# dotchen/LAV

Measured on AMD Instinct MI355X. Metric: frames/s full agent fwd (32k-pt LiDAR + 3 cams), higher is better.
Workload: dtype f32 (convolution contractions on the matrix cores with f32 accumulate at the error of an fp32 dot product, DESIGN 4.3: the layers on the split-operand kernel - BEV backbone, heads, crop stems, the brake net's mid-size layers - and ERFNet's persistent runs of pairs as two power-of-two-scaled fp16 pie

## Files before the change

### include/lav_amd.h

```cpp
#ifndef LAV_AMD_H
#define LAV_AMD_H

#include <stddef.h>
#include <stdint.h>

#ifdef __cplusplus
extern "C" {
#endif

#define LAV_ABI_VERSION 39

#define LAV_OK 0
#define LAV_EINVAL (-1)
#define LAV_EHIP (-2)
#define LAV_EWORKSPACE (-3)

int lav_abi_version(void);
const char *lav_last_error(void);
int lav_device_count(void);

int lav_profile_enable(int slots);
int lav_profile_reset(void);
int lav_profile_read(const char *kernel, double *total_ms, int *launches);

typedef struct lav_grid {
    float min_x, max_x, min_y, max_y;
    float ppm;
    int nx, ny;
} lav_grid;

typedef struct lav_pointnet {
    const float *w1, *b1, *w2, *b2;
    int num_input;
    int channels;
} lav_pointnet;

size_t lav_pillar_workspace_bytes(int batch, int max_points, const lav_grid *grid);
int lav_pillar_workspace_init(void *workspace, size_t workspace_bytes, void *stream);

int lav_pillar_scatter(const float *points, const int *h_num_points, int batch, int max_points, int D,
                       const lav_grid *grid, const lav_pointnet *net, float *canvas,
                       int *unique_coords, int *inverse, int *counts,
                       void *workspace, size_t workspace_bytes, void *stream);
int lav_pillar_amax_count(int batch, const lav_grid *grid);
int lav_pillar_scatter_amax(const float *points, const int *h_num_points, int batch, int max_points, int D,
                            const lav_grid *grid, const lav_pointnet *net, float *canvas,
                            int *unique_coords, int *inverse, int *counts, float *amax_parts,
                            void *workspace, size_t workspace_bytes, void *stream);

typedef struct lav_camera {
    float K[9];
    float l2w[16];
    float w2c[16];
} lav_camera;

int lav_paint(const float *lidar, int n, int lidar_dim, const float *sem, int ncam, int sem_c, int h, int w,
              const lav_camera *h_cams, float *fused, int *uvz, void *stream);

int lav_gru_cast(const float *embd, int B, int embd_dim, int H, int num_cmds, int T,
                 const float *w_ih, const float *w_hh, const float *b_ih, const float *b_hh,
                 const float *mlp_w, const float *mlp_b, float *out,
                 void *workspace, size_t workspace_bytes, void *stream);
size_t lav_gru_cast_workspace_bytes(int B, int embd_dim, int H, int num_cmds, int T);
// ... 136 lines not shown
int lav_bn_train_amax_count(int batch, int channels, long plane);
int lav_bn_train_forward_amax(const float *x, const float *residual, float *y, int batch, int channels, long plane, const float *gamma,
                              const float *beta, double eps, int relu_pre, int relu_post, float *save_mean, float *save_var,
                              float *save_rstd, float *amax_y, void *workspace, size_t workspace_bytes, void *stream);
int lav_bn_train_backward_amax(const float *x, const float *y, const float *dy, int batch, int channels, long plane, const float *gamma,
                               const float *save_mean, const float *save_rstd, int relu_pre, int relu_post, float *dx, float *dres,
                               float *dgamma, float *dbeta, float *amax_dx, void *workspace, size_t workspace_bytes, void *stream);

int lav_bn_train_forward_mask(const float *x, const float *residual, const float *chmask, float *y, int batch, int channels, long plane,
                              const float *gamma, const float *beta, double eps, int relu_post, float *save_mean, float *save_var,
                              float *save_rstd, float *amax_y, void *workspace, size_t workspace_bytes, void *stream);
int lav_bn_train_backward_mask(const float *x, const float *y, const float *dy, const float *chmask, int batch, int channels, long plane,
                               const float *gamma, const float *save_mean, const float *save_rstd, int relu_post, float *dx, float *dres,
                               float *dgamma, float *dbeta, float *amax_dx, void *workspace, size_t workspace_bytes, void *stream);

size_t lav_conv_wgrad_workspace_bytes(int batch, int cin, int cout, int h, int w, int ksize, int stride);
int lav_conv_wgrad(const float *x, const float *dy, int batch, int cin, int cout, int h, int w, int ksize, int stride, float *dw,
                   void *workspace, size_t workspace_bytes, void *stream);
int lav_conv_wgrad_amax(const float *x, const float *dy, int batch, int cin, int cout, int h, int w, int ksize, int stride, float *dw,
                        void *workspace, size_t workspace_bytes, const float *amax_x, int n_amax_x, const float *amax_dy, int n_amax_dy,
                        void *stream);

size_t lav_upconv_pointwise_packed_floats(int cin, int cout, int k);
int lav_upconv_pointwise_pack(int cin, int cout, int k, const float *h_weight, float *h_packed);
int lav_upconv_pointwise_parts(int batch, int cin, int cout, int ih, int iw, int k, int pad, int out_pad);
int lav_upconv_pointwise(int batch, int cin, int cout, int ih, int iw, int k, int pad, int out_pad, const float *x, const float *w_packed,
                         const float *scale, const float *shift, int relu_pre, int out_c_total, int out_c_offset, float *y,
                         float *amax_out, void *stream);

size_t lav_conv1d_pair_packed_weight_floats(int channels);
int lav_conv1d_pair_pack_weights(int channels, const float *h_weight, float *h_packed);
size_t lav_conv1d_pair_chain_workspace_bytes(int batch, int h);
size_t lav_conv1d_pair_chain_lds_bytes(int channels, int w, int d_b_max);
int lav_conv1d_pair_chain(int batch, int channels, int h, int w, int npairs, const int *d_a, const int *d_b, const int *residual,
                          const int *relu_post, const float *x, const float *const *wa_packed, const float *const *bias_a,
                          const float *const *wb_packed, const float *const *bias_b, const float *const *scale,
                          const float *const *shift, float *const *out, void *workspace, size_t workspace_bytes, void *stream);
int lav_conv1d_pair_chain_f16(int batch, int channels, int h, int w, int npairs, const int *d_a, const int *d_b, const int *residual,
                              const int *relu_post, const float *x, const float *const *wa_packed, const float *const *bias_a,
                              const float *const *wb_packed, const float *const *bias_b, const float *const *scale,
                              const float *const *shift, float *const *out, void *workspace, size_t workspace_bytes, void *stream);
int lav_conv1d_pair_chain_region(int row_offset, int clean_rows);
int lav_conv1d_pair_chain_status(const void *workspace, int *h_timeouts_launches2, void *stream);
size_t lav_conv1d_pair_lds_bytes(int channels, int w, int d_b);
size_t lav_conv3x3_run_f16_workspace_bytes(int channels, int h, int w, int nlayers);
size_t lav_conv3x3_run_f16_lds_bytes(int channels, int h, int w);
size_t lav_conv3x3_run_f16_weight_bytes(int channels);
int lav_conv3x3_run_f16_amax_count(int channels, int h, int w);
long lav_conv_f16_weights_offset(const lav_conv *c);
int lav_conv3x3_run_f16(int channels, int h, int w, int nlayers, const float *x, const void *const *w_f16, const float *const *scale,
                        const float *const *shift, float *out, const float *amax_in, int amax_in_count, float *amax_out, void *workspace,
                        size_t workspace_bytes, void *stream);
int lav_conv3x3_run_f16_status(const void *workspace, int *h_timeouts_launches2, void *stream);
int lav_conv1d_pair(int batch, int channels, int h, int w, int d_a, int d_b, const float *x, const float *wa_packed,
                    const float *bias_a, const float *wb_packed, const float *bias_b, const float *scale, const float *shift,
                    const float *residual, int relu_post, float *y, void *stream);

int lav_pool_affine(const float *x, int batch, int channels, int h, int w, const float *scale, const float *shift, int relu,
                    float *y, int out_c_total, int out_c_offset, void *stream);

int lav_pair_train_supported(int channels, int width);
size_t lav_pair_train_workspace_bytes(int batch, int channels, int h);
int lav_pair_train_forward(const float *x, const float *wa, const float *ba, const float *wb, const float *bb, int batch, int channels,
                           int h, int w, int dil, float *t, float *z, void *stream);
int lav_pair_train_backward(const float *x, const float *t, const float *dz, const float *wa, const float *wb, int batch, int channels,
                            int h, int w, int dil, float *dt, float *dx, float *dwa, float *dba, float *dwb, float *dbb, void *workspace,
                            size_t workspace_bytes, void *stream);

size_t lav_seg_xent_workspace_bytes(void);
int lav_seg_xent_forward(const float *logits, const long long *labels, int batch, int classes, long plane, float *loss, float *dlogits,
                         void *workspace, size_t workspace_bytes, void *stream);

int lav_seg_xent_up_forward(const float *logits, const void *labels, int label_bytes, int batch, int classes, int h, int w, int scale,
                            float *loss, float *dlogits, void *workspace, size_t workspace_bytes, void *stream);

typedef struct lav_camera_f64 {
    double l2w[16];
    double w2c[16];
    double K[9];
} lav_camera_f64;

int lav_paint_frames(const float *lidar, const int *offsets, int frames, int total, int lidar_dim, const float *sem, int ncam,
                     int sem_c, int h, int w, const lav_camera_f64 *h_cams, float *painted, int *uvz, void *stream);

int lav_image_u8_to_f32(const unsigned char *img, int n, int h, int w, int c_src, int reverse, float *out, void *stream);

enum { LAV_AUG_BLUR = 0, LAV_AUG_NOISE = 1, LAV_AUG_DROPOUT = 2, LAV_AUG_MULTIPLY = 3, LAV_AUG_CONTRAST = 4, LAV_AUG_GRAYSCALE = 5,
       LAV_AUG_ELASTIC = 6, LAV_AUG_OPS = 7 };

typedef struct lav_augment_params {
    int order[7];
    int active;
    int per_channel;
    unsigned sample;
    unsigned tag;
    float blur_sigma;
    float blur_w[5];
    float noise_scale;
    float dropout_p;
    float multiply[3];
    float contrast[3];
    float gray_alpha;
    float elastic_alpha;
    float field_w[5];
} lav_augment_params;

// ... 39 lines not shown
```

### lav_amd/_lib.py

```python
from __future__ import annotations

import ctypes as C
import os

HERE = os.path.dirname(os.path.abspath(__file__))
LIB_PATH = os.environ.get("LAV_AMD_LIB") or os.path.join(HERE, "liblav_amd.so")

ABI_VERSION = 39
MAX_CAM = 4
MAX_CAM_F64 = 8


class Grid(C.Structure):
    _fields_ = [("min_x", C.c_float), ("max_x", C.c_float), ("min_y", C.c_float), ("max_y", C.c_float),
                ("ppm", C.c_float), ("nx", C.c_int), ("ny", C.c_int)]


class PointNet(C.Structure):
    _fields_ = [("w1", C.c_void_p), ("b1", C.c_void_p), ("w2", C.c_void_p), ("b2", C.c_void_p),
                ("num_input", C.c_int), ("channels", C.c_int)]


class Camera(C.Structure):
    _fields_ = [("K", C.c_float * 9), ("l2w", C.c_float * 16), ("w2c", C.c_float * 16)]


class CameraF64(C.Structure):
    _fields_ = [("l2w", C.c_double * 16), ("w2c", C.c_double * 16), ("K", C.c_double * 9)]


class Conv(C.Structure):
    _fields_ = [(n, C.c_int) for n in (
        "batch", "in_c_total", "in_c_offset", "cin", "h", "w", "cout", "kh", "kw", "stride", "pad_h", "pad_w",
        "dil_h", "dil_w", "transposed", "out_pad", "out_c_total", "out_c_offset", "relu_pre", "relu_post", "sigmoid", "target_cus")] + [("pad_value", C.c_float), ("precision", C.c_int)]


CONV_F32, CONV_BF16X6, CONV_F16X3 = 1, 2, 3


_P, _I, _Z, _F = C.c_void_p, C.c_int, C.c_size_t, C.c_float
SIGNATURES = {
    "lav_abi_version": (_I, []),
    "lav_last_error": (C.c_char_p, []),
    "lav_device_count": (_I, []),
    "lav_profile_enable": (_I, [_I]),
    "lav_profile_reset": (_I, []),
    "lav_profile_read": (_I, [C.c_char_p, C.POINTER(C.c_double), C.POINTER(_I)]),
    "lav_pillar_workspace_bytes": (_Z, [_I, _I, C.POINTER(Grid)]),
    "lav_pillar_workspace_init": (_I, [_P, _Z, _P]),
    "lav_pillar_decorate_workspace_bytes": (_Z, [_I, _I, C.POINTER(Grid)]),
    "lav_pillar_scatter": (_I, [_P, C.POINTER(_I), _I, _I, _I, C.POINTER(Grid), C.POINTER(PointNet), _P, _P, _P, _P,
                                _P, _Z, _P]),
    "lav_pillar_amax_count": (_I, [_I, C.POINTER(Grid)]),
    "lav_pillar_scatter_amax": (_I, [_P, C.POINTER(_I), _I, _I, _I, C.POINTER(Grid), C.POINTER(PointNet), _P, _P, _P, _P, _P,
                                     _P, _Z, _P]),
    "lav_paint": (_I, [_P, _I, _I, _P, _I, _I, _I, _I, C.POINTER(Camera), _P, _P, _P]),
    "lav_paint_frames": (_I, [_P, _P, _I, _I, _I, _P, _I, _I, _I, _I, C.POINTER(CameraF64), _P, _P, _P]),
    "lav_image_u8_to_f32": (_I, [_P, _I, _I, _I, _I, _I, _P, _P]),
    "lav_gru_cast": (_I, [_P, _I, _I, _I, _I, _I, _P, _P, _P, _P, _P, _P, _P, _P, _Z, _P]),
    "lav_gru_cast_workspace_bytes": (_Z, [_I, _I, _I, _I, _I]),
    "lav_embed_cast": (_I, [_P, _I, _I, _I, _P, _I, _I, _I, _P, _P, _P, _P, _P, _P, _P, _P, _P, _P, _P, _P, _P]),
    "lav_gru_plan": (_I, [_P, _P, _P, _I, _I, _I, _I, _I, _I, _F, _F, _P, _P, _P, _P, _P, _P, _P, _P, _Z, _P]),
    "lav_gru_plan_steps": (_I, [_P, _P, _P, _I, _I, _I, _I, _I, _I, _F, _F, _P, _P, _P, _P, _P, _P, _P, _P, _Z, _P]),
    "lav_gru_plan_status": (_I, [_P, _Z, _I, _I, _I, _I, C.POINTER(_I), _P]),
    "lav_gru_plan_diag": (_I, [_P, _Z, _I, _I, _I, _I, C.POINTER(_I), _P]),
    "lav_gru_plan_workspace_bytes": (_Z, [_I, _I, _I, _I]),
    "lav_conv_out_hw": (_I, [C.POINTER(Conv), C.POINTER(_I), C.POINTER(_I)]),
    "lav_conv_packed_weight_floats": (_Z, [C.POINTER(Conv)]),
    "lav_conv_pack_weights": (_I, [C.POINTER(Conv), _P, _P]),
    "lav_conv_pack_map_ints": (_Z, [C.POINTER(Conv)]),
    "lav_conv_pack_map": (_I, [C.POINTER(Conv), _P]),
    "lav_conv_repack": (_I, [C.POINTER(Conv), _P, _P, _P, _P]),
    "lav_conv_repack_scratch": (_I, [C.POINTER(Conv), _P, _P, _P, _P, _Z, _P]),
    "lav_bn_fold": (_I, [_P, _P, _P, _P, C.c_double, _I, _P, _P, _P]),
    "lav_conv_wgrad_workspace_bytes": (_Z, [_I, _I, _I, _I, _I, _I, _I]),
    "lav_conv_wgrad": (_I, [_P, _P, _I, _I, _I, _I, _I, _I, _I, _P, _P, _Z, _P]),
    "lav_conv_wgrad_amax": (_I, [_P, _P, _I, _I, _I, _I, _I, _I, _I, _P, _P, _Z, _P, _I, _P, _I, _P]),
    "lav_absmax_parts": (_I, [_P, C.c_long, _P, _P]),
    "lav_conv_tile_info": (_I, [C.POINTER(Conv), C.POINTER(_I)]),
    "lav_conv_workspace_bytes": (_Z, [C.POINTER(Conv)]),
    "lav_conv2d": (_I, [C.POINTER(Conv), _P, _P, _P, _P, _P, _P, _P, _P, _Z, _P]),
    "lav_conv_amax_count": (_I, [C.POINTER(Conv)]),
    "lav_conv2d_amax": (_I, [C.POINTER(Conv), _P, _P, _P, _P, _P, _P, _P, _P, _Z, _P, _I, _P, _P]),
    "lav_deconv_grouped": (_I, [_I, _I, _I, _I, _I, C.POINTER(_I), _I, _I, _I, _I, _P, _P, _P, _I, _P, _P]),
    "lav_crop_rotate": (_I, [_P, _I, _I, _I, _I, _P, _P, _I, _F, _I, _F, _F, _P, _P]),
    "lav_crop_rotate_indexed": (_I, [_P, _I, _P, _I, _I, _I, _P, _P, _I, _F, _I, _F, _F, _P, _P]),
    "lav_crop_rotate_backward": (_I, [_P, _I, _P, _I, _I, _I, _P, _P, _I, _F, _I, _F, _F, _P, _P]),
    "lav_pillar_decorate": (_I, [_P, C.POINTER(_I), _I, _I, _I, C.POINTER(Grid), _P, _P, _P, _P, _P, _P, _Z, _P]),
    "lav_scatter_max": (_I, [_P, _P, _I, _I, _I, _P, _P, _P]),
    "lav_scatter_max_backward": (_I, [_P, _P, _I, _I, _I, _P, _P]),
    "lav_conv1d_pair_packed_weight_floats": (_Z, [_I]),
    "lav_conv1d_pair_pack_weights": (_I, [_I, _P, _P]),
    "lav_upconv_pointwise_packed_floats": (_Z, [_I, _I, _I]),
    "lav_upconv_pointwise_pack": (_I, [_I, _I, _I, _P, _P]),
    "lav_upconv_pointwise_parts": (_I, [_I] * 8),
    "lav_upconv_pointwise": (_I, [_I] * 8 + [_P, _P, _P, _P, _I, _I, _I, _P, _P, _P]),
    "lav_conv1d_pair_chain_workspace_bytes": (_Z, [_I, _I]),
    "lav_conv1d_pair_chain_region": (_I, [_I, _I]),
    "lav_conv1d_pair_chain_lds_bytes": (_Z, [_I, _I, _I]),
    "lav_conv1d_pair_chain": (_I, [_I, _I, _I, _I, _I, C.POINTER(_I), C.POINTER(_I), C.POINTER(_I), C.POINTER(_I), _P] + [C.POINTER(_P)] * 7 + [_P, _Z, _P]),
    "lav_conv1d_pair_chain_f16": (_I, [_I, _I, _I, _I, _I, C.POINTER(_I), C.POINTER(_I), C.POINTER(_I), C.POINTER(_I), _P] + [C.POINTER(_P)] * 7 + [_P, _Z, _P]),
    "lav_conv1d_pair_chain_status": (_I, [_P, C.POINTER(_I), _P]),
    "lav_conv1d_pair_lds_bytes": (_Z, [_I, _I, _I]),
    "lav_conv3x3_run_f16_workspace_bytes": (_Z, [_I, _I, _I, _I]),
    "lav_conv3x3_run_f16_lds_bytes": (_Z, [_I, _I, _I]),
    "lav_conv3x3_run_f16_weight_bytes": (_Z, [_I]),
    "lav_conv3x3_run_f16_amax_count": (_I, [_I, _I, _I]),
    "lav_conv_f16_weights_offset": (C.c_long, [C.POINTER(Conv)]),
    "lav_conv3x3_run_f16": (_I, [_I, _I, _I, _I, _P, C.POINTER(_P), C.POINTER(_P), C.POINTER(_P), _P, _P, _I, _P, _P, _Z, _P]),
    "lav_conv3x3_run_f16_status": (_I, [_P, C.POINTER(_I), _P]),
    "lav_conv1d_pair": (_I, [_I, _I, _I, _I, _I, _I, _P, _P, _P, _P, _P, _P, _P, _P, _I, _P, _P]),
    "lav_gru_seq_forward": (_I, [_P, _I, _P, _P, _P, _I, _I, _I, _P, _P, _P]),
    "lav_gru_seq_backward_workspace_bytes": (_Z, [_I, _I]),
    "lav_gru_seq_backward": (_I, [_P, _P, _P, _P, _P, _I, _I, _I, _P, _P, _P, _P, _Z, _P]),
    "lav_bn_train_workspace_bytes": (_Z, [_I]),
    "lav_bn_train_forward_mask": (_I, [_P, _P, _P, _P, _I, _I, C.c_long, _P, _P, C.c_double, _I, _P, _P, _P, _P, _P, _Z, _P]),
    "lav_bn_train_backward_mask": (_I, [_P, _P, _P, _P, _I, _I, C.c_long, _P, _P, _P, _I, _P, _P, _P, _P, _P, _P, _Z, _P]),
    "lav_pair_train_supported": (_I, [_I, _I]),
    "lav_pair_train_workspace_bytes": (_Z, [_I, _I, _I]),
    "lav_pair_train_forward": (_I, [_P, _P, _P, _P, _P, _I, _I, _I, _I, _I, _P, _P, _P]),
    "lav_pair_train_backward": (_I, [_P, _P, _P, _P, _P, _I, _I, _I, _I, _I, _P, _P, _P, _P, _P, _P, _P, _Z, _P]),
    "lav_seg_xent_workspace_bytes": (_Z, []),
    "lav_seg_xent_forward": (_I, [_P, _P, _I, _I, C.c_long, _P, _P, _P, _Z, _P]),
    "lav_seg_xent_up_forward": (_I, [_P, _P, _I, _I, _I, _I, _I, _I, _P, _P, _P, _Z, _P]),
    "lav_attn_train_workspace_bytes": (_Z, [_I, _I, _I, _I]),
    "lav_attn_train_forward": (_I, [_P, _I, _I, _I, _I, _P, _P, _P, _P, C.c_float, _P, _P, _P, _P, _P, _P]),
    "lav_attn_train_backward": (_I, [_P, _I, _I, _I, _I, _P, _P, _P, _P, C.c_float, _P, _P, _P, _P, _P, _P, _P, _P, _P, _Z, _P]),
    "lav_bn_train_forward": (_I, [_P, _P, _P, _I, _I, C.c_long, _P, _P, C.c_double, _I, _I, _P, _P, _P, _P, _Z, _P]),
    "lav_bn_train_backward": (_I, [_P, _P, _P, _I, _I, C.c_long, _P, _P, _P, _I, _I, _P, _P, _P, _P, _P, _Z, _P]),
    "lav_bn_train_amax_count": (_I, [_I, _I, C.c_long]),
    "lav_bn_train_forward_amax": (_I, [_P, _P, _P, _I, _I, C.c_long, _P, _P, C.c_double, _I, _I, _P, _P, _P, _P, _P, _Z, _P]),
    "lav_bn_train_backward_amax": (_I, [_P, _P, _P, _I, _I, C.c_long, _P, _P, _P, _I, _I, _P, _P, _P, _P, _P, _P, _Z, _P]),
    "lav_attn_pool": (_I, [_P, _I, _I, _I, _I, _P, _P, _P, _P, _P, _P]),
    "lav_linear_act": (_I, [_P, _I, _I, _P, _P, _I, _I, _P, _P]),
    "lav_maxpool3x3s2": (_I, [_P, _I, _I, _I, _I, _P, _P]),
    "lav_channel_affine": (_I, [_P, _I, _I, C.c_long, _P, _P, _P, _P]),
    "lav_nonfinite_count": (_I, [_I, C.POINTER(_P), C.POINTER(C.c_long), _P, _P]),
    "lav_copy_many": (_I, [_I, C.POINTER(_P), C.POINTER(_P), C.POINTER(_Z), _P]),
    "lav_stage_many": (_I, [_I, C.POINTER(_P), C.POINTER(_P), C.POINTER(_I), C.POINTER(C.c_long), C.POINTER(_I), _P]),
    "lav_det_decode": (_I, [_P, _I, _I, _I] + [C.c_double] * 10 + [_P, _P, _P]),
    "lav_det_decode_report": (_I, [_P, _I, _I, _I] + [C.c_double] * 10 + [_P, _P, _P, _P, _P, _P]),
    "lav_stage_many_block": (_I, [_I, C.POINTER(_P), C.POINTER(_P), C.POINTER(_I), C.POINTER(C.c_long), C.POINTER(_I), _P, _I, _P, _P]),
    "lav_batch_limit": (_I, [_P]),
    "lav_pool_affine": (_I, [_P, _I, _I, _I, _I, _P, _P, _I, _P, _I, _I, _P]),
    "lav_merge_ticks": (_I, [_P, _P, _I, _I, _P, _P]),
    "lav_stack_sweeps": (_I, [_P, _P, _P, _P, _P, _P, _I, _I, _I, _P, _P]),
    "lav_extract_peaks_workspace_bytes": (_Z, [_I, _I, _I]),
    "lav_extract_peaks": (_I, [_P, _I, _I, _I, _I, _I, _I, _P, _I, _P, _I, _P, _P, _Z, _P]),
    "lav_augment_u8": (_I, [_P, _P, _I, _I, _I, _P, C.c_ulonglong, _P]),
    "lav_bev_stack_u8": (_I, [_P, _P, _P, _P, _I, _I, _I, _I, _P]),
    "lav_bev_stack_tile_paths": (_I, [C.POINTER(C.c_double), C.POINTER(_I), _I, _I, C.POINTER(_I)]),
    "lav_debug_view": (_I, [_P, _I, _I, _P, _I, _I, _P, _I, _I, _P, _I, _P, _I, _P, _I, _P, _P, _P, C.c_double, C.c_double, _I, C.c_double, C.c_double, _I,
                            _I, _I, _P, _P, _P]),
    "lav_log_view": (_I, [_P, _I, _P, _I, _P, _P, _I, _I, _P, _P, _I, _P, _I, _I, _P, _P]),
    "lav_eval_acc_words": (_Z, [_I]),
    "lav_eval_frame": (_I, [_P, _P, _P, _I, _I, _F, _P, _I, _P, _P, _I, _I, _I, _P, _P, _I, _P, _P, _P, _I] + [C.c_double] * 6 + [_I, _P, _P]),
    "lav_eval_seg": (_I, [_P, _P, _I, _I, _I, _I, _I, _P, _P]),
    "lav_eval_scores": (_I, [_P, _P, _I, C.c_double, _I, _P, _P]),
    "lav_eval_plans_words": (_Z, [_I]),
    "lav_eval_plans": (_I, [_P, _P, _P, _P, _P, _P, _I, _I, _I, _P, _P, _P, _I, _P, _P]),
}

_lib = None
# ... 35 lines not shown
```

### lav_amd/build.py

```python
from __future__ import annotations

import os
import subprocess
import sys
import time

HERE = os.path.dirname(os.path.abspath(__file__))
REPO = os.path.dirname(HERE)
CSRC = os.path.join(HERE, "csrc")
LIB = os.path.join(HERE, "liblav_amd.so")
SOURCES = ["misc.hip", "pillar.hip", "paint.hip", "paint_frames.hip", "gru.hip", "gru_seq.hip", "conv.hip", "conv_f16.hip", "conv_pair.hip", "conv_run.hip", "deconv.hip", "crop.hip", "frame.hip", "attn.hip", "bn_train.hip", "conv_wgrad.hip", "upconv.hip", "conv_pair_train.hip", "augment.hip", "bev_stack.hip", "debug_view.hip", "log_view.hip", "eval_metrics.hip", "eval_camera.hip", "eval_plans.hip"]
EXTRA_FLAGS = {"pillar.hip": ["-ffp-contract=off"], "paint.hip": ["-ffp-contract=off"], "paint_frames.hip": ["-ffp-contract=off"], "crop.hip": ["-ffp-contract=off"],
               "frame.hip": ["-ffp-contract=off"], "augment.hip": ["-ffp-contract=off"], "bev_stack.hip": ["-ffp-contract=off"],
               "debug_view.hip": ["-ffp-contract=off", "-fhip-fp32-correctly-rounded-divide-sqrt"],
               "log_view.hip": ["-ffp-contract=off"],
               "eval_metrics.hip": ["-ffp-contract=off"],
               "eval_plans.hip": ["-ffp-contract=off"]}
FLAGS = ["--offload-arch=gfx950", "-O3", "-std=c++17", "-fPIC", "-Wall", "-Wno-unused-function", "-fno-slp-vectorize",
         "-I", os.path.join(REPO, "include"), "-I", CSRC]


def _hipcc() -> str:
    for c in (os.environ.get("HIPCC"), "/opt/rocm/bin/hipcc", "hipcc"):
        if c and (os.path.isabs(c) and os.path.exists(c) or not os.path.isabs(c)):
            return c
    raise RuntimeError("hipcc not found")


def needs_build() -> bool:
    if not os.path.exists(LIB):
        return True
    t = os.path.getmtime(LIB)
    deps = [os.path.join(CSRC, f) for f in os.listdir(CSRC)] + [os.path.join(REPO, "include", "lav_amd.h")]
    return any(os.path.getmtime(d) > t for d in deps)


def build(force: bool = False, verbose: bool = True) -> str:
    if not force and not needs_build():
        return LIB
    objs = []
    procs = []
    os.makedirs(os.path.join(HERE, "build"), exist_ok=True)
    t0 = time.time()
    for s in SOURCES:
        o = os.path.join(HERE, "build", s.replace(".hip", ".o"))
        objs.append(o)
        cmd = [_hipcc(), *FLAGS, *EXTRA_FLAGS.get(s, []), "-c", os.path.join(CSRC, s), "-o", o]
        procs.append((s, subprocess.Popen(cmd, stdout=subprocess.PIPE, stderr=subprocess.STDOUT, text=True)))
    for s, p in procs:
        out, _ = p.communicate()
        if p.returncode != 0:
            raise RuntimeError(f"hipcc failed on {s}:\n{out}")
        if verbose and out.strip():
            print(out)
    link = [_hipcc(), "--offload-arch=gfx950", "-shared", "-fPIC", *objs, "-o", LIB]
    r = subprocess.run(link, stdout=subprocess.PIPE, stderr=subprocess.STDOUT, text=True)
    if r.returncode != 0:
        raise RuntimeError("link failed:\n" + r.stdout)
    if verbose:
        print(f"built {LIB} in {time.time() - t0:.1f}s")
    return LIB


if __name__ == "__main__":
# ... 2 lines not shown
```

### lav_amd/lidar.py

```python
from __future__ import annotations

import torch
from torch import nn
import torch.nn.functional as F

from . import _lib
from . import ops
from .ops import Amax, ConvLayer, ConvRun, GroupedDeconv, PointwiseUpconv
from .point_pillar import PointPillarNet

_NORM = dict(eps=1e-3, momentum=0.01)


def _refreshable(obj):
    if isinstance(obj, dict):
        for v in obj.values():
            yield from _refreshable(v)
    elif isinstance(obj, (list, tuple)):
        for v in obj:
            yield from _refreshable(v)
    elif hasattr(obj, "refresh"):
        yield obj


class _Engine(nn.Module):

    def _drop(self):
        object.__setattr__(self, "_eng", None)
        object.__setattr__(self, "_stale", False)

    def _mark_stale(self):
        if self.__dict__.get("_eng") is not None:
            object.__setattr__(self, "_stale", True)

    def _tensor_ids(self):
        return tuple(id(t) for t in self.parameters()) + tuple(id(t) for t in self.buffers())

    def _fresh(self, device):
        eng = self.__dict__.get("_eng")
        if eng is None or eng.get("device") != device:
            return None
        if self.__dict__.get("_stale"):
            if eng["tensor_ids"] != self._tensor_ids():
                self._drop()
                return None
            for layer in _refreshable(eng):
                layer.refresh()
            object.__setattr__(self, "_stale", False)
        return eng

    def _apply(self, fn, *a, **k):
        self._drop()
        return super()._apply(fn, *a, **k)

    def train(self, mode: bool = True):
        if mode != self.training:
            self._mark_stale()
        return super().train(mode)

    def _load_from_state_dict(self, *a, **k):
        self._mark_stale()
# ... 11 lines not shown
def _stage(cin, cout, n):
    mods = []
    for j in range(n):
        mods += [nn.Conv2d(cin if j == 0 else cout, cout, 3, 2 if j == 0 else 1, 1, bias=False),
                 nn.ReLU(inplace=True), nn.BatchNorm2d(cout, **_NORM)]
    return nn.Sequential(*mods)


def _up(cin, cout, k, s, p=0, op=0):
    return nn.Sequential(nn.ConvTranspose2d(cin, cout, k, s, p, op, bias=False), nn.ReLU(inplace=True),
                         nn.BatchNorm2d(cout, **_NORM))


class ConvBackbone(_Engine):
    def __init__(self, num_feature=64, norm_cfg=None):
        super().__init__()
        f = num_feature
        self.conv1 = _stage(f, f, 4)
        self.conv2 = _stage(f, 2 * f, 6)
        self.conv3 = _stage(2 * f, 2 * f, 6)
        self.upconv1 = _up(f, 2 * f, 1, 1)
        self.upconv2 = _up(2 * f, 2 * f, 4, 2, 1)
        self.upconv3 = _up(2 * f, 2 * f, 4, 4, 1, 2)
        self.out_channels = 6 * f
        self._drop()

    def _engine(self, device):
        prec = ops.infer_precision()
        eng = self._fresh(device) or dict(device=device)
        key = ("backbone", prec)
        if key in eng:
            return eng[key]
        def stage(seq):
            out = []
            for j in range(0, len(seq), 3):
                conv, bn = seq[j], seq[j + 2]
                out.append(ConvLayer(conv.weight, stride=conv.stride[0], padding=conv.padding, bn=_bn_tuple(bn),
                                     bn_eps=bn.eps, relu_pre=True, precision=prec, device=device))
            return out
        ups = []
        off = 0
        for seq in (self.upconv1, self.upconv2, self.upconv3):
            ct, bn = seq[0], seq[2]
            if prec == _lib.CONV_F16X3 and PointwiseUpconv.takes(ct):
                ups.append(PointwiseUpconv(ct, bn, relu_pre=True, out_c_total=self.out_channels, out_c_offset=off, device=device))
            else:
                ups.append(ConvLayer(ct.weight, stride=ct.stride[0], padding=ct.padding, transposed=True,
                                     output_padding=ct.output_padding[0], bn=_bn_tuple(bn), bn_eps=bn.eps, relu_pre=True,
                                     out_c_total=self.out_channels, out_c_offset=off, precision=prec, device=device))
            off += ct.weight.shape[1]
        eng[key] = dict(s1=stage(self.conv1), s2=stage(self.conv2), s3=stage(self.conv3), ups=ups, amax={}, f16=prec == _lib.CONV_F16X3)
        want = ops.bev_run_stages() if prec == _lib.CONV_F16X3 else ()
        eng[key]["runs"] = [ConvRun(eng[key][s][1:]) if s in want and len(eng[key][s]) > 2 else None for s in ("s1", "s2", "s3")]
        eng["tensor_ids"] = self._tensor_ids()
        object.__setattr__(self, "_eng", eng)
        return eng[key]

    def forward_train(self, x):
        from .train.hipnn import conv_relu_bn
        f1 = conv_relu_bn(self.conv1, x)
        f2 = conv_relu_bn(self.conv2, f1)
        f3 = conv_relu_bn(self.conv3, f2)
        return torch.cat([conv_relu_bn(self.upconv1, f1), conv_relu_bn(self.upconv2, f2), conv_relu_bn(self.upconv3, f3)], dim=1)

    def forward(self, x, out=None):
        if self.training:
            return self.forward_train(x)
        self._need_eval()
        e = self._engine(x.device)
        if not e["f16"]:
            feats = []
            for st in (e["s1"], e["s2"], e["s3"]):
                for layer in st:
                    x = layer(x)
                feats.append(x)
            oh, ow = e["ups"][0].out_hw(feats[0].shape[2], feats[0].shape[3])
            if out is None:
                out = torch.empty((x.shape[0], self.out_channels, oh, ow), dtype=torch.float32, device=x.device)
            for up, f in zip(e["ups"], feats):
                up(f, out=out)
            return out
        B = x.shape[0]
        key = ops.amax_key(x)
        ams = e["amax"].get(key)
        if ams is None:
            ams = e["amax"][key] = [Amax(x.device) for _ in range(len(e["s1"]) + len(e["s2"]) + len(e["s3"]) + 1)]
        stages = (e["s1"], e["s2"], e["s3"])
        feats, feat_am, am_prev, i = [], [], ops.amax_of(x), 0
        for si, st in enumerate(stages):
            run, li = e["runs"][si], 0
            while li < len(st):
                layer = st[li]
                oh, ow = layer.out_hw(x.shape[2], x.shape[3])
                runs_next = run is not None and run.takes(B, oh, ow)
                n = len(st) - 1 if runs_next and li == 1 else 1
                nxt = li + n
                readers = ([run if runs_next and nxt == 1 else st[nxt]] if nxt < len(st) else ([stages[si + 1][0]] if si + 1 < len(stages) else [])) + \
                          ([e["ups"][si]] if nxt == len(st) else [])
                am = ams[i + n - 1].reset() if any(r.uses_amax(B, oh, ow) for r in readers) else None
                x = (run if n > 1 else layer)(x, amax_in=am_prev, amax_out=am)
                am_prev, i, li = am, i + n, nxt
            feats.append(x); feat_am.append(am_prev)
        oh, ow = e["ups"][0].out_hw(feats[0].shape[2], feats[0].shape[3])
        if out is None:
            out = torch.empty((B, self.out_channels, oh, ow), dtype=torch.float32, device=x.device)
        am_out = ams[-1].reset()
# ... 111 lines not shown
```

### lav_amd/ops.py

```python
from __future__ import annotations

import ctypes as C
import os as _os
import threading as _threading
from typing import Optional, Sequence

import numpy as np
import torch

from . import _lib
from ._lib import Camera, Conv, Grid, PointNet, check

_workspaces: dict = {}


def _stream() -> int:
    return torch.cuda.current_stream().cuda_stream


def _ptr(t: Optional[torch.Tensor]) -> Optional[int]:
    return None if t is None else t.data_ptr()


def _f32c(t: torch.Tensor, name: str) -> torch.Tensor:
# ... 1118 lines not shown

class ConvRun:

    def __init__(self, layers):
        lib = _lib.load()
        layers = list(layers)
        l0 = layers[0]
        for l in layers:
            d = l.desc
            if not (d.precision == _lib.CONV_F16X3 and (d.kh, d.kw, d.stride, d.pad_h, d.pad_w, d.dil_h, d.dil_w) == (3, 3, 1, 1, 1, 1, 1)
                    and not d.transposed and l.cin == l.cout == l0.cin and l.in_c_total == l.cin and l.out_c_total == l.cout
                    and l.bias is None and l.scale is not None and d.relu_pre and not d.relu_post and not d.sigmoid and d.pad_value == 0.0):
                raise RuntimeError("ConvRun: layers must be identical conv3x3 / ReLU / BatchNorm layers packed for LAV_CONV_F16X3")
        self.layers, self.ch = layers, l0.cin
        probe = Conv.from_buffer_copy(l0.desc)
        probe.h, probe.w = 64, 64
        self._woff = int(lib.lav_conv_f16_weights_offset(C.byref(probe)))
        if self._woff < 0 or len(layers) > 8:
            raise RuntimeError("ConvRun: at most 8 layers with fp16 packed weights")
        n = len(layers)
        self._n = n

    def takes(self, B: int, h: int, w: int) -> bool:
        return B == 1 and _lib.load().lav_conv3x3_run_f16_workspace_bytes(self.ch, h, w, self._n) > 0

    def uses_amax(self, B: int, h: int, w: int) -> bool:
        return self.takes(B, h, w)

    def __call__(self, x: torch.Tensor, out: Optional[torch.Tensor] = None, amax_in: Optional["Amax"] = None,
                 amax_out: Optional["Amax"] = None) -> torch.Tensor:
        lib = _lib.load()
        x = _f32c(x, "x")
        B, ch, h, w = x.shape
        if ch != self.ch or not self.takes(B, h, w):
            raise RuntimeError(f"ConvRun: input {tuple(x.shape)} is not served (lav_conv3x3_run_f16_workspace_bytes)")
        if out is None:
            out = torch.empty_like(x)
        n = self._n
        ws = _workspace(("conv_run", id(self), ch, h, w), lib.lav_conv3x3_run_f16_workspace_bytes(ch, h, w, n), x.device)
        if amax_in is not None and amax_in.count > 0:
            a_in, n_in = amax_in.buf, amax_in.count
        else:
            a_in = _workspace(("conv_run_amax", id(self)), 512 * 4, x.device).view(torch.float32)
            n_in = 512
            check(lib.lav_absmax_parts(_ptr(x), x.numel(), _ptr(a_in), _stream()), "lav_absmax_parts")
        a_out = amax_out.take(lib.lav_conv3x3_run_f16_amax_count(ch, h, w)) if amax_out is not None else None
        pa = lambda ts: (C.c_void_p * n)(*[t if isinstance(t, int) else t.data_ptr() for t in ts])
        check(lib.lav_conv3x3_run_f16(ch, h, w, n, _ptr(x), pa([l.w.data_ptr() + 4 * self._woff for l in self.layers]),
                                      pa([l.scale for l in self.layers]), pa([l.shift for l in self.layers]), _ptr(out), _ptr(a_in), n_in,
                                      _ptr(a_out), _ptr(ws), ws.numel(), _stream()), "lav_conv3x3_run_f16")
        return out


def bev_run_status(device, stream=None):
    st = stream if stream is not None else torch.cuda.current_stream()
    device = torch.device(device)
    if device.index is None:
        device = torch.device("cuda", torch.cuda.current_device())
    tot = [0, 0]
    for (key, dev, s), ws in list(_workspaces.items()):
        if isinstance(key, tuple) and key and key[0] == "conv_run" and dev == device and s == st.cuda_stream:
            v = (C.c_int * 2)()
            check(_lib.load().lav_conv3x3_run_f16_status(_ptr(ws), v, st.cuda_stream), "lav_conv3x3_run_f16_status")
            tot[0] += int(v[0]); tot[1] += int(v[1])
    return tuple(tot)


_CU_COUNT = {}


def _cu_count(device) -> int:
    idx = torch.device(device).index
    idx = torch.cuda.current_device() if idx is None else idx
    if idx not in _CU_COUNT:
        _CU_COUNT[idx] = torch.cuda.get_device_properties(idx).multi_processor_count
    return _CU_COUNT[idx]


train_work = {"crop_rotate_backward_bytes": 0, "crop_rotate_backward_calls": 0, "gru_seq_forward_flops": 0, "gru_seq_backward_flops": 0,
              "bn_train_fwd_bytes": 0, "bn_train_bwd_bytes": 0, "conv_wgrad_flops": 0}


class _CropRotateIndexed(torch.autograd.Function):

    @staticmethod
    def forward(ctx, features, map_index, locs, oris, ppm, crop, ox, oy):
        lib = _lib.load()
        features = _f32c(features, "features")
        locs, oris = _f32c(locs.detach().reshape(-1, 2), "locs"), _f32c(oris.detach().reshape(-1), "oris")
        if map_index.dtype != torch.int32 or not map_index.is_cuda:
            raise RuntimeError("crop_rotate_indexed: map_index must be an int32 tensor in HBM")
        M, Cc, H, W = features.shape
        n = locs.shape[0]
        out = torch.empty((n, Cc, crop, crop), dtype=torch.float32, device=features.device)
        check(lib.lav_crop_rotate_indexed(_ptr(features), M, _ptr(map_index), Cc, H, W, _ptr(locs), _ptr(oris), n, float(ppm), int(crop),
                                          float(ox), float(oy), _ptr(out), _stream()), "lav_crop_rotate_indexed")
        ctx.save_for_backward(map_index, locs, oris)
        ctx.geom = (M, Cc, H, W, float(ppm), int(crop), float(ox), float(oy))
        return out

    @staticmethod
    def backward(ctx, grad_out):
        map_index, locs, oris = ctx.saved_tensors
        M, Cc, H, W, ppm, crop, ox, oy = ctx.geom
        grad_out = _f32c(grad_out, "grad_out")
        grad_feat = torch.empty((M, Cc, H, W), dtype=torch.float32, device=grad_out.device)
# ... 202 lines not shown
```

Measured before the change: 524.3.

## Fuse BEV backbone 3x3 conv stages into halo-tiled single-kernel f16 MFMA runs

Adds a new kernel that runs up to three consecutive 64-channel 3x3 conv+ReLU+BN layers on one spatial tile per workgroup. Each layer's intermediate activations stay in LDS as split fp16 pieces, and the kernel recomputes halo regions instead of writing them to global memory. The BEV backbone stages that have no persistent run assigned now use this path by default for batch 1. The aim is to cut the global-memory round trips and launches between layers. In exchange it spends extra compute on overlapping halos, uses heavy LDS and registers, and derives a per-tile amax for rescaling between layers.

```diff
diff --git a/include/lav_amd.h b/include/lav_amd.h
--- a/include/lav_amd.h
+++ b/include/lav_amd.h
@@ -8,7 +8,7 @@
 extern "C" {
 #endif
 
-#define LAV_ABI_VERSION 39
+#define LAV_ABI_VERSION 40
 
 #define LAV_OK 0
 #define LAV_EINVAL (-1)
@@ -251,6 +251,10 @@
                         const float *const *shift, float *out, const float *amax_in, int amax_in_count, float *amax_out, void *workspace,
                         size_t workspace_bytes, void *stream);
 int lav_conv3x3_run_f16_status(const void *workspace, int *h_timeouts_launches2, void *stream);
+size_t lav_conv3x3_tile_f16_lds_bytes(int channels, int h, int w, int nlayers);
+int lav_conv3x3_tile_f16_amax_count(int channels, int h, int w, int nlayers);
+int lav_conv3x3_tile_f16(int channels, int h, int w, int nlayers, const float *x, const void *const *w_f16, const float *const *scale,
+                         const float *const *shift, float *out, const float *amax_in, int amax_in_count, float *amax_out, void *stream);
 int lav_conv1d_pair(int batch, int channels, int h, int w, int d_a, int d_b, const float *x, const float *wa_packed,
                     const float *bias_a, const float *wb_packed, const float *bias_b, const float *scale, const float *shift,
                     const float *residual, int relu_post, float *y, void *stream);
diff --git a/lav_amd/_lib.py b/lav_amd/_lib.py
--- a/lav_amd/_lib.py
+++ b/lav_amd/_lib.py
@@ -6,7 +6,7 @@
 HERE = os.path.dirname(os.path.abspath(__file__))
 LIB_PATH = os.environ.get("LAV_AMD_LIB") or os.path.join(HERE, "liblav_amd.so")
 
-ABI_VERSION = 39
+ABI_VERSION = 40
 MAX_CAM = 4
 MAX_CAM_F64 = 8
 
@@ -109,6 +109,9 @@
     "lav_conv_f16_weights_offset": (C.c_long, [C.POINTER(Conv)]),
     "lav_conv3x3_run_f16": (_I, [_I, _I, _I, _I, _P, C.POINTER(_P), C.POINTER(_P), C.POINTER(_P), _P, _P, _I, _P, _P, _Z, _P]),
     "lav_conv3x3_run_f16_status": (_I, [_P, C.POINTER(_I), _P]),
+    "lav_conv3x3_tile_f16_lds_bytes": (_Z, [_I, _I, _I, _I]),
+    "lav_conv3x3_tile_f16_amax_count": (_I, [_I, _I, _I, _I]),
+    "lav_conv3x3_tile_f16": (_I, [_I, _I, _I, _I, _P, C.POINTER(_P), C.POINTER(_P), C.POINTER(_P), _P, _P, _I, _P, _P]),
     "lav_conv1d_pair": (_I, [_I, _I, _I, _I, _I, _I, _P, _P, _P, _P, _P, _P, _P, _P, _I, _P, _P]),
     "lav_gru_seq_forward": (_I, [_P, _I, _P, _P, _P, _I, _I, _I, _P, _P, _P]),
     "lav_gru_seq_backward_workspace_bytes": (_Z, [_I, _I]),
diff --git a/lav_amd/build.py b/lav_amd/build.py
--- a/lav_amd/build.py
+++ b/lav_amd/build.py
@@ -9,7 +9,7 @@
 REPO = os.path.dirname(HERE)
 CSRC = os.path.join(HERE, "csrc")
 LIB = os.path.join(HERE, "liblav_amd.so")
-SOURCES = ["misc.hip", "pillar.hip", "paint.hip", "paint_frames.hip", "gru.hip", "gru_seq.hip", "conv.hip", "conv_f16.hip", "conv_pair.hip", "conv_run.hip", "deconv.hip", "crop.hip", "frame.hip", "attn.hip", "bn_train.hip", "conv_wgrad.hip", "upconv.hip", "conv_pair_train.hip", "augment.hip", "bev_stack.hip", "debug_view.hip", "log_view.hip", "eval_metrics.hip", "eval_camera.hip", "eval_plans.hip"]
+SOURCES = ["misc.hip", "pillar.hip", "paint.hip", "paint_frames.hip", "gru.hip", "gru_seq.hip", "conv.hip", "conv_f16.hip", "conv_pair.hip", "conv_run.hip", "conv_tile.hip", "deconv.hip", "crop.hip", "frame.hip", "attn.hip", "bn_train.hip", "conv_wgrad.hip", "upconv.hip", "conv_pair_train.hip", "augment.hip", "bev_stack.hip", "debug_view.hip", "log_view.hip", "eval_metrics.hip", "eval_camera.hip", "eval_plans.hip"]
 EXTRA_FLAGS = {"pillar.hip": ["-ffp-contract=off"], "paint.hip": ["-ffp-contract=off"], "paint_frames.hip": ["-ffp-contract=off"], "crop.hip": ["-ffp-contract=off"],
                "frame.hip": ["-ffp-contract=off"], "augment.hip": ["-ffp-contract=off"], "bev_stack.hip": ["-ffp-contract=off"],
                "debug_view.hip": ["-ffp-contract=off", "-fhip-fp32-correctly-rounded-divide-sqrt"],
diff --git a/lav_amd/csrc/conv_tile.hip b/lav_amd/csrc/conv_tile.hip
--- /dev/null
+++ b/lav_amd/csrc/conv_tile.hip
@@ -0,0 +1,286 @@
+#include <cstdlib>
+#include <cstring>
+
+#include "common.hpp"
+#include "split_arith.hpp"
+
+namespace {
+using namespace lav;
+
+constexpr int TILE_C = 64, TILE_MAX_L = 3, TILE_MAX_WG = 16384;
+constexpr size_t TILE_W_BYTES = (size_t)9 * (TILE_C / 32) * (TILE_C / 16) * 2 * 1024;
+
+struct TileArgs {
+    const float *x;
+    float *out;
+    const unsigned char *w[TILE_MAX_L];
+    const float *wscale[TILE_MAX_L], *scale[TILE_MAX_L], *shift[TILE_MAX_L];
+    const float *amax_in;
+    float *amax_out;
+    int amax_in_count, H, W, tiles_x;
+};
+
+__device__ __forceinline__ void tile_load_w(const unsigned char *p, int t, u32x4 (&dst)[2]) {
+    dst[0] = *reinterpret_cast<const u32x4 *>(p + t * (TILE_C / 16) * 2048);
+    dst[1] = *reinterpret_cast<const u32x4 *>(p + t * (TILE_C / 16) * 2048 + 1024);
+}
+
+template <int NA, int RWI, int NPI>
+__device__ __forceinline__ void tile_mma(const unsigned char *in, const int (&base)[2], int half, u32x4 (&wr)[9][2], const unsigned char *w_this,
+                                         const unsigned char *w_next, f32x16 (&tot)[2]) {
+    constexpr int PIECE = 8 * NPI * 16;
+#pragma nounroll
+    for (int ch = 0; ch < TILE_C / 16; ++ch) {
+        f32x16 acc[NA];
+#pragma unroll
+        for (int j = 0; j < NA; ++j)
+#pragma unroll
+            for (int r = 0; r < 16; ++r) acc[j][r] = 0.f;
+        const unsigned char *w_refill = ch + 1 < TILE_C / 16 ? w_this + (ch + 1) * 2048 : w_next;
+        const unsigned char *bin = in + (ch * 2 + half) * NPI * 16;
+#pragma unroll
+        for (int t = 0; t < 9; ++t) {
+            const int toff = ((t / 3) * RWI + (t % 3)) * 16;
+            u32x4 b[NA][2];
+#pragma unroll
+            for (int j = 0; j < NA; ++j) {
+                b[j][0] = *reinterpret_cast<const u32x4 *>(bin + toff + base[j]);
+                b[j][1] = *reinterpret_cast<const u32x4 *>(bin + PIECE + toff + base[j]);
+            }
+#pragma unroll
+            for (int j = 0; j < NA; ++j)
+                acc[j] = __builtin_amdgcn_mfma_f32_32x32x16_f16(__builtin_bit_cast(f16x8, wr[t][1]), __builtin_bit_cast(f16x8, b[j][0]), acc[j], 0, 0, 0);
+#pragma unroll
+            for (int j = 0; j < NA; ++j)
+                acc[j] = __builtin_amdgcn_mfma_f32_32x32x16_f16(__builtin_bit_cast(f16x8, wr[t][0]), __builtin_bit_cast(f16x8, b[j][1]), acc[j], 0, 0, 0);
+#pragma unroll
+            for (int j = 0; j < NA; ++j)
+                acc[j] = __builtin_amdgcn_mfma_f32_32x32x16_f16(__builtin_bit_cast(f16x8, wr[t][0]), __builtin_bit_cast(f16x8, b[j][0]), acc[j], 0, 0, 0);
+            tile_load_w(w_refill, t, wr[t]);
+        }
+#pragma unroll
+        for (int j = 0; j < NA; ++j)
+#pragma unroll
+            for (int r = 0; r < 16; ++r) tot[j][r] += acc[j][r];
+    }
+}
+
+template <int OH, int OW, bool LAST>
+__device__ __forceinline__ float tile_layer(const TileArgs &a, const unsigned char *in, unsigned char *outb, int oy0, int ox0, float sx, float sw,
+                                            const float *s_epi, float *s_wmax, u32x4 (&wr)[9][2], const unsigned char *w_this,
+                                            const unsigned char *w_next) {
+    constexpr int NP = OH * OW, NB = (NP + 31) / 32, RWI = OW + 2, NPI = (OH + 2) * (OW + 2);
+    static_assert(NB <= 8, "two pixel blocks per wave group at the most");
+    const int tid = threadIdx.x, lane = tid & 63, l31 = lane & 31, half = lane >> 5;
+    const int wid = __builtin_amdgcn_readfirstlane(tid >> 6);
+    const int cbw = wid & 1, grp = wid >> 1;
+    const int H = a.H, W = a.W;
+    const long plane = (long)H * W;
+
+    int qu[2], base[2];
+#pragma unroll
+    for (int j = 0; j < 2; ++j) {
+        qu[j] = (grp + 4 * j) * 32 + l31;
+        const int q = min(qu[j], NP - 1);
+        base[j] = ((q / OW) * RWI + (q % OW)) * 16;
+    }
+    const int nact = grp + 4 < NB ? 2 : grp < NB ? 1 : 0;
+    f32x16 acc[2];
+#pragma unroll
+    for (int j = 0; j < 2; ++j)
+#pragma unroll
+        for (int r = 0; r < 16; ++r) acc[j][r] = 0.f;
+    if (nact == 2) tile_mma<2, RWI, NPI>(in, base, half, wr, w_this, w_next, acc);
+    else tile_mma<1, RWI, NPI>(in, base, half, wr, w_this, w_next, acc);
+
+    float out_sx, out_sw;
+    f16_out_scales(sx, sw, out_sx, out_sw);
+    float lm = 0.f;
+    bool inmap[2];
+#pragma unroll
+    for (int j = 0; j < 2; ++j) {
+        const int q = min(qu[j], NP - 1);
+        const int gy = oy0 + q / OW, gx = ox0 + q % OW;
+        inmap[j] = j < nact && qu[j] < NP && gy >= 0 && gy < H && gx >= 0 && gx < W;
+        float *yo = a.out + (long)gy * W + gx;
+#pragma unroll
+        for (int r = 0; r < 16; ++r) {
+            const int co = cbw * 32 + (r & 3) + 8 * (r >> 2) + 4 * half;
+            float vv = acc[j][r] * out_sx * out_sw;
+            vv = vv > 0.f ? vv : 0.f;
+            vv = fmaf(vv, s_epi[co], s_epi[64 + co]);
+            vv = inmap[j] ? vv : 0.f;
+            if (LAST) {
+                if (inmap[j]) yo[co * plane] = vv;
+            } else {
+                acc[j][r] = vv;
+            }
+            lm = fmaxf(lm, finite_abs(vv));
+        }
+    }
+    lm = wave_finite_absmax(lm);
+    if (lane == 0) s_wmax[wid] = lm;
+    __syncthreads();
+    float m = 0.f;
+#pragma unroll
+    for (int i = 0; i < 8; ++i) m = fmaxf(m, s_wmax[i]);
+    if (LAST) {
+        if (tid == 0 && a.amax_out) a.amax_out[blockIdx.x] = m;
+        return 0.f;
+    }
+    const float sn = f16_scale_of(m), inv = 1.f / sn;
+#pragma unroll
+    for (int j = 0; j < 2; ++j) {
+        if (j < nact && qu[j] < NP) {
+#pragma unroll
+            for (int g = 0; g < 4; ++g) {
+                unsigned p00, p01, p10, p11;
+                split2h_pair(acc[j][4 * g] * inv, acc[j][4 * g + 1] * inv, p00, p10);
+                split2h_pair(acc[j][4 * g + 2] * inv, acc[j][4 * g + 3] * inv, p01, p11);
+                unsigned char *d = outb + ((cbw * 4 + g) * NP + qu[j]) * 16 + half * 8;
+                *reinterpret_cast<u32x2 *>(d) = u32x2{p00, p01};
+                lds_store_fence();
+                *reinterpret_cast<u32x2 *>(d + 8 * NP * 16) = u32x2{p10, p11};
+                lds_store_fence();
+            }
+        }
+    }
+    __syncthreads();
+    return sn;
+}
+
+template <int TH, int TW, int L>
+__global__ __launch_bounds__(512) void k_conv3x3_tile_f16(TileArgs a) {
+    extern __shared__ __attribute__((aligned(16))) unsigned char smem[];
+    constexpr int RH = TH + 2 * L, RW = TW + 2 * L, NPA = RH * RW;
+    constexpr int NPB = L > 1 ? (TH + 2 * (L - 1)) * (TW + 2 * (L - 1)) : 0;
+    constexpr int BUF_A = 2 * 8 * NPA * 16, BUF_B = 2 * 8 * NPB * 16;
+    unsigned char *bufA = smem, *bufB = smem + BUF_A;
+    float *s_epi = reinterpret_cast<float *>(smem + BUF_A + BUF_B);
+    float *s_wmax = s_epi + L * 128;
+    const int tid = threadIdx.x, lane = tid & 63;
+    const int wid = __builtin_amdgcn_readfirstlane(tid >> 6);
+    const int H = a.H, W = a.W;
+    const long plane = (long)H * W;
+    const int ty0 = (blockIdx.x / a.tiles_x) * TH, tx0 = (blockIdx.x % a.tiles_x) * TW;
+
+    u32x4 wr[9][2];
+    const long wlane = (long)(wid & 1) * 9 * (TILE_C / 16) * 2048 + lane * 16;
+#pragma unroll
+    for (int t = 0; t < 9; ++t) tile_load_w(a.w[0] + wlane, t, wr[t]);
+    if (tid < L * 128) {
+        const int l = tid >> 7, c = tid & 63;
+        s_epi[tid] = (tid & 64) ? a.shift[l][c] : a.scale[l][c];
+    }
+    const float m_in = parts_absmax(a.amax_in, a.amax_in_count, lane);
+    float sx = f16_scale_of(m_in);
+
+    {
+        constexpr int NTASK = NPA * 8, NTK = (NTASK + 511) / 512;
+        const float inv = 1.f / sx;
+        float v[NTK][8];
+        bool ok[NTK];
+#pragma unroll
+        for (int u = 0; u < NTK; ++u) {
+            const int task = min(tid + u * 512, NTASK - 1);
+            const int g = task / NPA, p = task - g * NPA;
+            const int gy = ty0 - L + p / RW, gx = tx0 - L + p % RW;
+            ok[u] = gy >= 0 && gy < H && gx >= 0 && gx < W;
+            const float *sp = a.x + (long)g * 8 * plane + (long)min(max(gy, 0), H - 1) * W + min(max(gx, 0), W - 1);
+#pragma unroll
+            for (int c = 0; c < 8; ++c) v[u][c] = sp[c * plane];
+        }
+#pragma unroll
+        for (int u = 0; u < NTK; ++u) {
+            const int task = tid + u * 512;
+            if (task < NTASK) {
+                u32x4 q0, q1;
+#pragma unroll
+                for (int e = 0; e < 4; ++e) {
+                    unsigned p0, p1;
+                    split2h_pair(ok[u] ? v[u][2 * e] * inv : 0.f, ok[u] ? v[u][2 * e + 1] * inv : 0.f, p0, p1);
+                    q0[e] = p0; q1[e] = p1;
+                }
+                *reinterpret_cast<u32x4 *>(bufA + task * 16) = q0;
+                *reinterpret_cast<u32x4 *>(bufA + BUF_A / 2 + task * 16) = q1;
+            }
+        }
+    }
+    __syncthreads();
+
+    if constexpr (L == 1) {
+        tile_layer<TH, TW, true>(a, bufA, nullptr, ty0, tx0, sx, *a.wscale[0], s_epi, s_wmax, wr, a.w[0] + wlane, a.w[0] + wlane);
+    } else if constexpr (L == 2) {
+        sx = tile_layer<TH + 2, TW + 2, false>(a, bufA, bufB, ty0 - 1, tx0 - 1, sx, *a.wscale[0], s_epi, s_wmax, wr, a.w[0] + wlane, a.w[1] + wlane);
+        tile_layer<TH, TW, true>(a, bufB, nullptr, ty0, tx0, sx, *a.wscale[1], s_epi + 128, s_wmax, wr, a.w[1] + wlane, a.w[1] + wlane);
+    } else {
+        sx = tile_layer<TH + 4, TW + 4, false>(a, bufA, bufB, ty0 - 2, tx0 - 2, sx, *a.wscale[0], s_epi, s_wmax, wr, a.w[0] + wlane, a.w[1] + wlane);
+        sx = tile_layer<TH + 2, TW + 2, false>(a, bufB, bufA, ty0 - 1, tx0 - 1, sx, *a.wscale[1], s_epi + 128, s_wmax, wr, a.w[1] + wlane, a.w[2] + wlane);
+        tile_layer<TH, TW, true>(a, bufA, nullptr, ty0, tx0, sx, *a.wscale[2], s_epi + 256, s_wmax, wr, a.w[2] + wlane, a.w[2] + wlane);
+    }
+}
+
+struct TileConfig { int th, tw, tiles_x, tiles; size_t lds; };
+
+bool tile_config(int channels, int h, int w, int nlayers, TileConfig &c) {
+    if (channels != TILE_C || nlayers < 1 || nlayers > TILE_MAX_L || h < 1 || w < 1 || h > 32768 || w > 32768) return false;
+    static const bool tall = [] { const char *e = getenv("LAV_BEV_TILE_SHAPE"); return e && !strcmp(e, "16x8"); }();
+    c.th = tall ? 16 : 8; c.tw = tall ? 8 : 16;
+    c.tiles_x = (w + c.tw - 1) / c.tw;
+    const long tiles = (long)c.tiles_x * ((h + c.th - 1) / c.th);
+    if (tiles > TILE_MAX_WG) return false;
+    c.tiles = (int)tiles;
+    const int L = nlayers;
+    const size_t npa = (size_t)(c.th + 2 * L) * (c.tw + 2 * L), npb = L > 1 ? (size_t)(c.th + 2 * (L - 1)) * (c.tw + 2 * (L - 1)) : 0;
+    c.lds = (npa + npb) * 2 * 8 * 16 + (size_t)L * 128 * 4 + 8 * 4;
+    return c.lds <= 160 * 1024;
+}
+
+template <int TH, int TW, int L>
+int tile_launch(const TileArgs &a, const TileConfig &c, hipStream_t st) {
+    static bool attr = false;
+    if (!attr) {
+        LAV_HIP(hipFuncSetAttribute(reinterpret_cast<const void *>(&k_conv3x3_tile_f16<TH, TW, L>), hipFuncAttributeMaxDynamicSharedMemorySize, 160 * 1024));
+        attr = true;
+    }
+    hipLaunchKernelGGL((k_conv3x3_tile_f16<TH, TW, L>), dim3(c.tiles), dim3(512), c.lds, st, a);
+    return LAV_OK;
+}
+}
+
+extern "C" size_t lav_conv3x3_tile_f16_lds_bytes(int channels, int h, int w, int nlayers) {
+    TileConfig c;
+    return tile_config(channels, h, w, nlayers, c) ? c.lds : 0;
+}
+
+extern "C" int lav_conv3x3_tile_f16_amax_count(int channels, int h, int w, int nlayers) {
+    TileConfig c;
+    return tile_config(channels, h, w, nlayers, c) ? c.tiles : 0;
+}
+
+extern "C" int lav_conv3x3_tile_f16(int channels, int h, int w, int nlayers, const float *x, const void *const *w_f16, const float *const *scale,
+                                    const float *const *shift, float *out, const float *amax_in, int amax_in_count, float *amax_out, void *stream) {
+    TileConfig c;
+    LAV_REQUIRE(tile_config(channels, h, w, nlayers, c), "lav_conv3x3_tile_f16: %d layers of %d channels on %d x %d are not served (lav_conv3x3_tile_f16_lds_bytes returns 0)",
+                nlayers, channels, h, w);
+    LAV_REQUIRE(x && w_f16 && scale && shift && out && amax_in && amax_in_count >= 1, "lav_conv3x3_tile_f16: null argument (the first layer's scale comes from amax_in)");
+    TileArgs a;
+    for (int i = 0; i < TILE_MAX_L; ++i) {
+        const int j = i < nlayers ? i : nlayers - 1;
+        LAV_REQUIRE(w_f16[j] && scale[j] && shift[j], "lav_conv3x3_tile_f16: null argument of layer %d", j);
+        a.w[i] = static_cast<const unsigned char *>(w_f16[j]);
+        a.wscale[i] = reinterpret_cast<const float *>(a.w[i] + TILE_W_BYTES);
+        a.scale[i] = scale[j]; a.shift[i] = shift[j];
+    }
+    a.x = x; a.out = out; a.amax_in = amax_in; a.amax_in_count = amax_in_count; a.amax_out = amax_out;
+    a.H = h; a.W = w; a.tiles_x = c.tiles_x;
+    hipStream_t st = static_cast<hipStream_t>(stream);
+    const int tok = timer_begin("conv3x3_tile", st);
+    int rc;
+    if (c.th == 8) rc = nlayers == 1 ? tile_launch<8, 16, 1>(a, c, st) : nlayers == 2 ? tile_launch<8, 16, 2>(a, c, st) : tile_launch<8, 16, 3>(a, c, st);
+    else rc = nlayers == 1 ? tile_launch<16, 8, 1>(a, c, st) : nlayers == 2 ? tile_launch<16, 8, 2>(a, c, st) : tile_launch<16, 8, 3>(a, c, st);
+    if (rc != LAV_OK) return rc;
+    timer_end(tok, st);
+    LAV_LAUNCH_CHECK();
+    return LAV_OK;
+}
diff --git a/lav_amd/lidar.py b/lav_amd/lidar.py
--- a/lav_amd/lidar.py
+++ b/lav_amd/lidar.py
@@ -6,7 +6,7 @@
 
 from . import _lib
 from . import ops
-from .ops import Amax, ConvLayer, ConvRun, GroupedDeconv, PointwiseUpconv
+from .ops import Amax, ConvLayer, ConvRun, ConvTileRun, GroupedDeconv, PointwiseUpconv
 from .point_pillar import PointPillarNet
 
 _NORM = dict(eps=1e-3, momentum=0.01)
@@ -124,6 +124,11 @@
         eng[key] = dict(s1=stage(self.conv1), s2=stage(self.conv2), s3=stage(self.conv3), ups=ups, amax={}, f16=prec == _lib.CONV_F16X3)
         want = ops.bev_run_stages() if prec == _lib.CONV_F16X3 else ()
         eng[key]["runs"] = [ConvRun(eng[key][s][1:]) if s in want and len(eng[key][s]) > 2 else None for s in ("s1", "s2", "s3")]
+        if prec == _lib.CONV_F16X3 and ops.bev_tile_enabled():
+            for i, s in enumerate(("s1", "s2", "s3")):
+                st = eng[key][s]
+                if eng[key]["runs"][i] is None and 2 < len(st) <= 4 and st[1].cin == 64:
+                    eng[key]["runs"][i] = ConvTileRun(st[1:])
         eng["tensor_ids"] = self._tensor_ids()
         object.__setattr__(self, "_eng", eng)
         return eng[key]
diff --git a/lav_amd/ops.py b/lav_amd/ops.py
--- a/lav_amd/ops.py
+++ b/lav_amd/ops.py
@@ -1194,6 +1194,42 @@
         return out
 
 
+def bev_tile_enabled() -> bool:
+    return _os.environ.get("LAV_BEV_TILE", BEV_TILE_DEFAULT).strip().lower() not in ("0", "", "off", "none")
+
+
+BEV_TILE_DEFAULT = "1"
+
+
+class ConvTileRun(ConvRun):
+
+    def takes(self, B: int, h: int, w: int) -> bool:
+        return B == 1 and _lib.load().lav_conv3x3_tile_f16_lds_bytes(self.ch, h, w, self._n) > 0
+
+    def __call__(self, x: torch.Tensor, out: Optional[torch.Tensor] = None, amax_in: Optional["Amax"] = None,
+                 amax_out: Optional["Amax"] = None) -> torch.Tensor:
+        lib = _lib.load()
+        x = _f32c(x, "x")
+        B, ch, h, w = x.shape
+        if ch != self.ch or not self.takes(B, h, w):
+            raise RuntimeError(f"ConvTileRun: input {tuple(x.shape)} is not served (lav_conv3x3_tile_f16_lds_bytes)")
+        if out is None:
+            out = torch.empty_like(x)
+        n = self._n
+        if amax_in is not None and amax_in.count > 0:
+            a_in, n_in = amax_in.buf, amax_in.count
+        else:
+            a_in = _workspace(("conv_run_amax", id(self)), 512 * 4, x.device).view(torch.float32)
+            n_in = 512
+            check(lib.lav_absmax_parts(_ptr(x), x.numel(), _ptr(a_in), _stream()), "lav_absmax_parts")
+        a_out = amax_out.take(lib.lav_conv3x3_tile_f16_amax_count(ch, h, w, n)) if amax_out is not None else None
+        pa = lambda ts: (C.c_void_p * n)(*[t if isinstance(t, int) else t.data_ptr() for t in ts])
+        check(lib.lav_conv3x3_tile_f16(ch, h, w, n, _ptr(x), pa([l.w.data_ptr() + 4 * self._woff for l in self.layers]),
+                                       pa([l.scale for l in self.layers]), pa([l.shift for l in self.layers]), _ptr(out), _ptr(a_in), n_in,
+                                       _ptr(a_out), _stream()), "lav_conv3x3_tile_f16")
+        return out
+
+
 def bev_run_status(device, stream=None):
     st = stream if stream is not None else torch.cuda.current_stream()
     device = torch.device(device)
```

Result: faster. 535.6, median of 6 (+2.2%).
